# chenjiaoAngel/Paddle-Lite

Hardware: AMD Instinct MI355X
Metric: INT8 images/sec MobileNetV1 224x224 (higher is better)
Workload: dtype int8; 1 GPU; MobileNetV1 INT8 full graph 224x224 (27 int8 convs + pool + fc + softmax), random-init weights, 128 images per step and GPU (4 predictors / HIP streams, each running whole steps: 4 steps in flight), input resident in HBM; steps_in_flight=4, global_batch=128

## Files before the change

paddle-lite_amd/csrc/conv_stem_common.h:

```cpp
#pragma once
#include <type_traits>

#include "gemm_epilogue.h"
#include "gemm_tr_common.h"
#include "plhip_kernels.h"

namespace plhip {

constexpr int STEM_LDS_PITCH = 272;

inline dim3 stem_grid(const DirectS2Args& a) {
  const long nblk = (long)(((a.ow >> 2) + 31) / 32) * ((a.oh + 3) / 4) * a.n;
  return dim3((unsigned)((nblk + 7) / 8 * 8));
}

template <class F>
inline void stem_dispatch(const DirectS2Args& a, int out, F&& launch) {
  using std::integral_constant;
  const bool mfull = a.cout % 32 == 0;
#define PLHIP_STEM(O)                                                                \
  do {                                                                               \
    if (mfull) launch(integral_constant<int, O>{}, integral_constant<bool, true>{}); \
    else launch(integral_constant<int, O>{}, integral_constant<bool, false>{});      \
  } while (0)
  if (out == OUT_I32) PLHIP_STEM(OUT_I32);
  else if (out == OUT_F32) PLHIP_STEM(OUT_F32);
  else PLHIP_STEM(OUT_I8);
#undef PLHIP_STEM
}

__device__ __forceinline__ bool stem_block(const DirectS2Args& a, int& bx, int& by, int& b) {
  const int nx = ((a.ow >> 2) + 31) >> 5, ny = (a.oh + 3) >> 2;
  const unsigned nb = (unsigned)(nx * ny * a.n), per = (nb + 7) >> 3;
  const unsigned vb = (blockIdx.x & 7) * per + (blockIdx.x >> 3);
  bx = (int)(vb % (unsigned)nx);
  const unsigned t = vb / (unsigned)nx;
  by = (int)(t % (unsigned)ny);
  b = (int)(t / (unsigned)ny);
  return vb < nb;
}

template <bool TAIL>
__device__ __forceinline__ void stem_gemm_args(const DirectS2Args& a, GemmArgs& g) {
  g.y = a.y;
  g.scale = a.scale;
  g.bias = a.bias;
  g.M = a.cout;
  g.HWY = a.oh * a.ow;
  g.y_bstride = (size_t)a.cout * a.oh * a.ow;
  g.act = a.act;
  g.alpha = a.alpha;
  g.res = TAIL ? a.res : nullptr;
  g.res_relu = TAIL ? a.res_relu : 0;
  g.y2 = TAIL ? a.y2 : nullptr;
  g.inv_scale2 = TAIL ? a.inv_scale2 : 0.f;
}

template <int OUT>
__device__ __forceinline__ v4i stem3x3_begin(const DirectS2Args& a, const int8_t* __restrict__ afrag, int lane, float* lsb,
                                             GemmArgs& g) {
  stem_gemm_args<false>(a, g);
  const v4i af0 = *reinterpret_cast<const v4i*>(afrag + (size_t)lane * 16);
  if (OUT != OUT_I32) stage_scale_bias<1, OUT>(g, 0, lane, lsb);
  return af0;
}

__device__ __forceinline__ void stem3x3_lds_windows(const uint8_t* img, int cin, int lane, int wave, uint32_t (&win)[4][5]) {
  const int c = lane & 31, h = lane >> 5;
#pragma unroll
  for (int L = 0; L < 5; ++L) {
    const int cr = 5 * h + L;
    const int ci = cr / 3, r3 = cr - ci * 3;
    const bool live = cr < 3 * cin;
    const int lrow = live ? ci * 9 + 2 * wave + r3 : 0;
    const uint8_t* p = img + lrow * STEM_LDS_PITCH + 8 * c;
    const v2i lo = *reinterpret_cast<const v2i*>(p), hi = *reinterpret_cast<const v2i*>(p + 8);
    const uint32_t m = live ? 0xffffffffu : 0u;
    const uint32_t d0 = (uint32_t)lo[0] & m, d1 = (uint32_t)lo[1] & m, d2 = (uint32_t)hi[0] & m, d3 = (uint32_t)hi[1] & m;
    win[0][L] = __builtin_amdgcn_alignbyte(d1, d0, 3);
    win[1][L] = __builtin_amdgcn_alignbyte(d2, d1, 1);
    win[2][L] = __builtin_amdgcn_alignbyte(d2, d1, 3);
    win[3][L] = __builtin_amdgcn_alignbyte(d3, d2, 1);
  }
}

template <int OUT, bool MFULL>
__device__ __forceinline__ void stem3x3_mfma(const GemmArgs g, const int8_t* __restrict__ afrag, v4i af0, const uint32_t (&win)[4][5],
                                             float* lsb, int lane, int b, int hw, bool qvalid) {
  const int h = lane >> 5;
  v4i bf[4];
#pragma unroll
  for (int j = 0; j < 4; ++j) {
    bf[j][0] = (int)__builtin_amdgcn_perm(win[j][1], win[j][0], 0x04020100u);
    bf[j][1] = (int)__builtin_amdgcn_perm(win[j][2], win[j][1], 0x05040201u);
    bf[j][2] = (int)__builtin_amdgcn_perm(win[j][3], win[j][2], 0x06050402u);
    bf[j][3] = (int)(win[j][4] & 0x00ffffffu);
  }
  const int MT = (g.M + 31) >> 5;
  for (int mt = 0; mt < MT; ++mt) {
    v4i af = af0;
    if (mt > 0) {
      af = *reinterpret_cast<const v4i*>(afrag + ((size_t)mt * 64 + lane) * 16);
      if (OUT != OUT_I32) stage_scale_bias<1, OUT>(g, mt, lane, lsb);
    }
    v16i acc[1][4];
    const v16i zero16 = {0, 0, 0, 0, 0, 0, 0, 0, 0, 0, 0, 0, 0, 0, 0, 0};
#pragma unroll
    for (int j = 0; j < 4; ++j) acc[0][j] = __builtin_amdgcn_mfma_i32_32x32x32_i8(af, bf[j], zero16, 0, 0, 0);
    if (qvalid) gemm_epilogue_act<1, OUT, true, MFULL>(g, acc, mt, h, b, hw, lsb, g.HWY - hw);
  }
}

template <int OUT, bool MFULL>
__device__ __forceinline__ void stem3x3_staged(const DirectS2Args& a, const int8_t* __restrict__ afrag, const uint8_t* img, float* lsb,
                                               int lane, int wave, int bx, int by, int b) {
  const int owq = a.ow >> 2;
  const int oy = by * 4 + wave;
  int xq = bx * 32 + (lane & 31);
  const bool qvalid = xq < owq && oy < a.oh;
  if (xq >= owq) xq = owq - 1;

  GemmArgs g;
  const v4i af0 = stem3x3_begin<OUT>(a, afrag, lane, lsb, g);
  __syncthreads();

  uint32_t win[4][5];
  stem3x3_lds_windows(img, a.cin, lane, wave, win);
  stem3x3_mfma<OUT, MFULL>(g, afrag, af0, win, lsb, lane, b, oy * a.ow + 4 * xq, qvalid);
}

}
```

paddle-lite_amd/csrc/conv_stem_f32in.hip:

```cpp
#include "conv_stem_common.h"

namespace plhip {

bool conv3x3s2_f32in_supported(const DirectS2Args& a) {
  return a.cin >= 1 && a.cin <= 3 && (a.ow & 3) == 0 && (a.w & 3) == 0 && a.pl == 1 && (a.pt == 0 || a.pt == 1) && a.cout <= 128 &&
         (long)a.n * a.cin * a.h * a.w < (1L << 31) && (long)(((a.ow >> 2) + 31) / 32) * ((a.oh + 3) / 4) * a.n < (1L << 31) - 8;
}

template <int OUT, bool MFULL>
__global__ __launch_bounds__(256) void conv3x3s2_mfma_f32in_kernel(DirectS2Args a, const int8_t* __restrict__ afrag) {
  PLHIP_PRELOAD(a.xf); PLHIP_PRELOAD(a.y); PLHIP_PRELOAD(a.scale); PLHIP_PRELOAD(a.bias); PLHIP_PRELOAD(afrag);
  PLHIP_PRELOAD(a.n); PLHIP_PRELOAD(a.cin); PLHIP_PRELOAD(a.h); PLHIP_PRELOAD(a.w); PLHIP_PRELOAD(a.cout); PLHIP_PRELOAD(a.oh);
  PLHIP_PRELOAD(a.ow); PLHIP_PRELOAD(a.pt); PLHIP_PRELOAD(a.act); PLHIP_PRELOAD(a.alpha); PLHIP_PRELOAD(a.x_inv_scale);
  __shared__ __attribute__((aligned(16))) float lsb_all[4][64];
  __shared__ __attribute__((aligned(16))) uint8_t img[27 * STEM_LDS_PITCH];
  const int lane = threadIdx.x & 63;
  const int wave = __builtin_amdgcn_readfirstlane((int)(threadIdx.x >> 6));
  float* lsb = lsb_all[wave];
  int bx, by, b;
  if (!stem_block(a, bx, by, b)) return;

  const int c0 = 256 * bx - 4, ih0 = 8 * by - a.pt;
  const int nrows = a.cin * 9;
  const float inv = a.x_inv_scale;
  const size_t img_base = (size_t)b * a.cin * a.h * a.w;
  constexpr int NPIECE = (27 * 66 + 255) / 256;
  v4f pv[NPIECE];
  int pdst[NPIECE];
#pragma unroll
  for (int it = 0; it < NPIECE; ++it) {
    const int k = it * 256 + (int)threadIdx.x;
    const int row = k / 66, piece = k - row * 66;
    const int ci = row / 9, j = row - ci * 9;
    const int ih = ih0 + j, col = c0 + 4 * piece;
    pdst[it] = k < nrows * 66 ? row * STEM_LDS_PITCH + 4 * piece : -1;
    pv[it] = v4f{0.f, 0.f, 0.f, 0.f};
    if (k < nrows * 66 && ih >= 0 && ih < a.h && col >= 0 && col < a.w)
      pv[it] = *reinterpret_cast<const v4f*>(a.xf + img_base + ((size_t)ci * a.h + ih) * a.w + col);
  }
#pragma unroll
  for (int it = 0; it < NPIECE; ++it) {
    const v4f v = pv[it];
    const uint32_t pk = pack4_i8(round_sat_i8(inv * v[0]), round_sat_i8(inv * v[1]), round_sat_i8(inv * v[2]), round_sat_i8(inv * v[3]));
    if (pdst[it] >= 0) *reinterpret_cast<uint32_t*>(img + pdst[it]) = pk;
  }

  stem3x3_staged<OUT, MFULL>(a, afrag, img, lsb, lane, wave, bx, by, b);
}

void launch_conv3x3s2_f32in(const DirectS2Args& a, const int8_t* afrag, int out, hipStream_t s) {
  stem_dispatch(a, out, [&](auto O, auto MF) {
    hipLaunchKernelGGL((conv3x3s2_mfma_f32in_kernel<decltype(O)::value, decltype(MF)::value>), stem_grid(a), dim3(256), 0, s, a, afrag);
  });
}

}
```

paddle-lite_amd/csrc/conv_stem_u8in.hip:

```cpp
#include "conv_stem_common.h"

namespace plhip {

bool conv3x3s2_u8in_supported(const DirectS2Args& a, const ImageArgs& im) {
  return conv3x3s2_f32in_supported(a) && (im.cs == 1 || im.cs == 3 || im.cs == 4) && im.c == (im.cs == 1 ? 1 : 3) && a.cin == im.c &&
         im.n == a.n && im.h == a.h && im.w == a.w && (long)a.n * a.h * a.w * im.cs < (1L << 31);
}

template <int OUT, bool MFULL, int CS>
__global__ __launch_bounds__(256) void conv3x3s2_mfma_u8in_kernel(DirectS2Args a, ImageArgs im, const int8_t* __restrict__ afrag) {
  PLHIP_PRELOAD(im.src); PLHIP_PRELOAD(a.y); PLHIP_PRELOAD(a.scale); PLHIP_PRELOAD(a.bias); PLHIP_PRELOAD(afrag);
  PLHIP_PRELOAD(a.n); PLHIP_PRELOAD(a.cin); PLHIP_PRELOAD(a.h); PLHIP_PRELOAD(a.w); PLHIP_PRELOAD(a.cout); PLHIP_PRELOAD(a.oh);
  PLHIP_PRELOAD(a.ow); PLHIP_PRELOAD(a.pt); PLHIP_PRELOAD(a.act); PLHIP_PRELOAD(a.alpha); PLHIP_PRELOAD(a.x_inv_scale);
  constexpr int C = CS == 1 ? 1 : 3;
  __shared__ __attribute__((aligned(16))) float lsb_all[4][64];
  __shared__ __attribute__((aligned(16))) uint8_t img[27 * STEM_LDS_PITCH];
  const int lane = threadIdx.x & 63;
  const int wave = __builtin_amdgcn_readfirstlane((int)(threadIdx.x >> 6));
  float* lsb = lsb_all[wave];
  int bx, by, b;
  if (!stem_block(a, bx, by, b)) return;

  const int c0 = 256 * bx - 4, ih0 = 8 * by - a.pt;
  const float inv = a.x_inv_scale;
  constexpr int NPIECE = (9 * 66 + 255) / 256;
  uint32_t pw[NPIECE][CS];
  int pdst[NPIECE];
  bool pin[NPIECE];
#pragma unroll
  for (int it = 0; it < NPIECE; ++it) {
    const int k = it * 256 + (int)threadIdx.x;
    const int j = k / 66, piece = k - j * 66;
    const int ih = ih0 + j, col = c0 + 4 * piece;
    pdst[it] = k < 9 * 66 ? j * STEM_LDS_PITCH + 4 * piece : -1;
    pin[it] = k < 9 * 66 && ih >= 0 && ih < a.h && col >= 0 && col < a.w;
#pragma unroll
    for (int d = 0; d < CS; ++d) pw[it][d] = 0u;
    if (pin[it]) {
      const uint32_t* p = reinterpret_cast<const uint32_t*>(im.src + (((size_t)b * a.h + ih) * a.w + col) * CS);
#pragma unroll
      for (int d = 0; d < CS; ++d) pw[it][d] = p[d];
    }
  }
#pragma unroll
  for (int it = 0; it < NPIECE; ++it) {
#pragma unroll
    for (int ci = 0; ci < C; ++ci) {
      int q[4];
#pragma unroll
      for (int e = 0; e < 4; ++e) {
        const int bi = e * CS + ci;
        const float u = (float)((pw[it][bi >> 2] >> (8 * (bi & 3))) & 0xffu);
        q[e] = round_sat_i8(inv * ((u - im.mean[ci]) * im.scale[ci]));
      }
      const uint32_t pk = pin[it] ? pack4_i8(q[0], q[1], q[2], q[3]) : 0u;
      if (pdst[it] >= 0) *reinterpret_cast<uint32_t*>(img + ci * 9 * STEM_LDS_PITCH + pdst[it]) = pk;
    }
  }

  stem3x3_staged<OUT, MFULL>(a, afrag, img, lsb, lane, wave, bx, by, b);
}

template <int CS>
static void launch_u8in_cs(const DirectS2Args& a, const ImageArgs& im, const int8_t* afrag, int out, hipStream_t s) {
  stem_dispatch(a, out, [&](auto O, auto MF) {
    hipLaunchKernelGGL((conv3x3s2_mfma_u8in_kernel<decltype(O)::value, decltype(MF)::value, CS>), stem_grid(a), dim3(256), 0, s, a, im, afrag);
  });
}

void launch_conv3x3s2_u8in(const DirectS2Args& a, const ImageArgs& im, const int8_t* afrag, int out, hipStream_t s) {
  if (im.cs == 1) launch_u8in_cs<1>(a, im, afrag, out, s);
  else if (im.cs == 3) launch_u8in_cs<3>(a, im, afrag, out, s);
  else launch_u8in_cs<4>(a, im, afrag, out, s);
}

}
```

paddle-lite_amd/csrc/misc_ops.hip:

```cpp
#include <stdlib.h>

#include "plhip_device.h"
#include "plhip_kernels.h"

namespace plhip {

__device__ __forceinline__ float mul_then_add_two_roundings(float a, float s, float b) {
#pragma clang fp contract(off)
  const float p = a * s;
  return p + b;
}
__device__ __forceinline__ float fc_epilogue_f32(int acc, float s, float b, int flags) {
  float y = (flags & 2) ? mul_then_add_two_roundings((float)acc, s, b) : __fmaf_rn((float)acc, s, b);
  if (flags & 1) y = y > 0.f ? y : 0.f;
  return y;
}

__global__ void pack_fc_kernel(const int8_t* __restrict__ w, int8_t* __restrict__ wp, int k, int n) {
  const int k4n = (k + 3) / 4;
  const size_t total = (size_t)k4n * n * 4;
  for (size_t idx = (size_t)blockIdx.x * blockDim.x + threadIdx.x; idx < total; idx += (size_t)gridDim.x * blockDim.x) {
    const int j = idx & 3;
    const size_t t = idx >> 2;
    const int col = (int)(t % n);
    const int kq = (int)(t / n);
    const int kk = kq * 4 + j;
    wp[idx] = kk < k ? w[(size_t)kk * n + col] : (int8_t)0;
  }
}

#define FC_MB 8
template <int OUT>
__global__ __launch_bounds__(256) void fc_i8_kernel(const int8_t* __restrict__ x, const int8_t* __restrict__ wp,
                                                    const float* __restrict__ scale, const float* __restrict__ bias,
                                                    void* __restrict__ y, int m, int k, int n, int relu) {
  const int col = blockIdx.x * 256 + threadIdx.x;
  const int m0 = blockIdx.y * FC_MB;
  const int k4n = (k + 3) / 4;
  int acc[FC_MB];
#pragma unroll
  for (int i = 0; i < FC_MB; ++i) acc[i] = 0;
  const int colc = col < n ? col : n - 1;
  const uint32_t* wq = reinterpret_cast<const uint32_t*>(wp) + colc;
  for (int kq = 0; kq < k4n; ++kq) {
    const int wv = (int)wq[(size_t)kq * n];
#pragma unroll
    for (int i = 0; i < FC_MB; ++i) {
      const int mi = m0 + i < m ? m0 + i : m - 1;
      const int8_t* xr = x + (size_t)mi * k + kq * 4;
      uint32_t xv = 0;
      if (kq * 4 + 3 < k) {
        __builtin_memcpy(&xv, xr, 4);
      } else {
        for (int j = 0; j < 4; ++j)
          if (kq * 4 + j < k) xv |= (uint32_t)(uint8_t)xr[j] << (8 * j);
      }
      acc[i] = __builtin_amdgcn_sdot4((int)xv, wv, acc[i], false);
    }
  }
  if (col >= n) return;
  const float s = (OUT == OUT_I32) ? 1.f : scale[col];
  const float bi = (OUT != OUT_I32 && bias) ? bias[col] : 0.f;
#pragma unroll
  for (int i = 0; i < FC_MB; ++i) {
    if (m0 + i >= m) break;
    const size_t off = (size_t)(m0 + i) * n + col;
    if (OUT == OUT_I32) {
      reinterpret_cast<int*>(y)[off] = acc[i];
    } else {
      const float f = fc_epilogue_f32(acc[i], s, bi, relu);
      if (OUT == OUT_F32) reinterpret_cast<float*>(y)[off] = f;
      else reinterpret_cast<int8_t*>(y)[off] = (int8_t)round_sat_i8(f);
    }
  }
}

#define FCF_MB 16
template <int OUT>
__global__ __launch_bounds__(256) void fc_i8_fast_kernel(const int8_t* __restrict__ x, const int8_t* __restrict__ wp,
                                                         const float* __restrict__ scale, const float* __restrict__ bias,
                                                         void* __restrict__ y, int m, int k, int n, int relu) {
  extern __shared__ __attribute__((aligned(16))) uint8_t fsm[];
  const int lane = threadIdx.x & 63;
  const int wave = __builtin_amdgcn_readfirstlane(threadIdx.x >> 6);
  const int col = blockIdx.x * 64 + lane;
  const int m0 = blockIdx.y * FCF_MB;
  const int k4n = k >> 2;
  const int k16n = k >> 4;
  {
    const v4i* src = reinterpret_cast<const v4i*>(x);
    v4i* dst = reinterpret_cast<v4i*>(fsm);
    for (int i = threadIdx.x; i < FCF_MB * k16n; i += 256) {
      const int r = i / k16n, c16 = i - r * k16n;
      const int mi = m0 + r < m ? m0 + r : m - 1;
      dst[i] = src[(size_t)mi * k16n + c16];
    }
  }
  __syncthreads();
  const int g0 = (k16n * wave) / 4, g1 = (k16n * (wave + 1)) / 4;
  const int colc = col < n ? col : n - 1;
  const uint32_t* wq = reinterpret_cast<const uint32_t*>(wp) + colc;
  int acc[FCF_MB];
#pragma unroll
  for (int i = 0; i < FCF_MB; ++i) acc[i] = 0;
  for (int gq = g0; gq < g1; ++gq) {
    int wv[4];
#pragma unroll
    for (int u = 0; u < 4; ++u) wv[u] = (int)wq[(size_t)(gq * 4 + u) * n];
#pragma unroll
    for (int i = 0; i < FCF_MB; ++i) {
      const v4i xv = *reinterpret_cast<const v4i*>(fsm + ((size_t)i * k16n + gq) * 16);
#pragma unroll
      for (int u = 0; u < 4; ++u) acc[i] = __builtin_amdgcn_sdot4(xv[u], wv[u], acc[i], false);
    }
  }
  __syncthreads();
  int* red = reinterpret_cast<int*>(fsm);
#pragma unroll
  for (int i = 0; i < FCF_MB; ++i) red[(wave * FCF_MB + i) * 64 + lane] = acc[i];
  __syncthreads();
  if (col >= n) return;
  const float s = (OUT == OUT_I32) ? 1.f : scale[col];
  const float bi = (OUT != OUT_I32 && bias) ? bias[col] : 0.f;
#pragma unroll
  for (int j = 0; j < FCF_MB / 4; ++j) {
    const int i = wave * (FCF_MB / 4) + j;
    if (m0 + i >= m) break;
    const int a = red[(0 * FCF_MB + i) * 64 + lane] + red[(1 * FCF_MB + i) * 64 + lane] + red[(2 * FCF_MB + i) * 64 + lane] +
                  red[(3 * FCF_MB + i) * 64 + lane];
    const size_t off = (size_t)(m0 + i) * n + col;
    if (OUT == OUT_I32) {
      reinterpret_cast<int*>(y)[off] = a;
    } else {
      const float f = fc_epilogue_f32(a, s, bi, relu);
      if (OUT == OUT_F32) reinterpret_cast<float*>(y)[off] = f;
      else reinterpret_cast<int8_t*>(y)[off] = (int8_t)round_sat_i8(f);
    }
  }
}

size_t fc_dot4_bytes(int k, int n) { return (((size_t)((k + 3) / 4) * n * 4) + 15) & ~(size_t)15; }
size_t fc_packed_bytes(int k, int n) { return fc_dot4_bytes(k, n) + (size_t)((n + 31) / 32) * ((k + 31) / 32) * 1024; }

__global__ void pack_fc_mfma_kernel(const int8_t* __restrict__ w, int8_t* __restrict__ wp, int k, int n) {
  const int KS = (k + 31) / 32;
  const size_t total = (size_t)((n + 31) / 32) * KS * 1024;
  for (size_t idx = (size_t)blockIdx.x * blockDim.x + threadIdx.x; idx < total; idx += (size_t)gridDim.x * blockDim.x) {
    const int j = idx & 15, lane = (idx >> 4) & 63;
    const size_t t = idx >> 10;
    const int ks = (int)(t % KS), nt = (int)(t / KS);
    const int nn = nt * 32 + (lane & 31), kk = ks * 32 + 16 * (lane >> 5) + j;
    wp[idx] = (nn < n && kk < k) ? w[(size_t)kk * n + nn] : (int8_t)0;
  }
}

template <int OUT>
__global__ __launch_bounds__(256) void fc_i8_mfma_kernel(const int8_t* __restrict__ x, const int8_t* __restrict__ wfrag,
                                                         const float* __restrict__ scale, const float* __restrict__ bias,
                                                         void* __restrict__ y, int m, int k, int n, int relu) {
  __shared__ int red[4][16][64];
  const int lane = threadIdx.x & 63;
  const int wave = __builtin_amdgcn_readfirstlane((int)(threadIdx.x >> 6));
  const int c = lane & 31, h = lane >> 5;
  const int nt = blockIdx.x, mt = blockIdx.y;
  const int KS = k >> 5;
  const int ks0 = (KS * wave) >> 2, ks1 = (KS * (wave + 1)) >> 2;
  const int mrow = mt * 32 + c < m ? mt * 32 + c : m - 1;
  const int8_t* xb = x + (size_t)mrow * k + 16 * h;
  const int8_t* ab = wfrag + (size_t)nt * KS * 1024 + lane * 16;
  const int n0 = nt * 32 + 8 * wave + 4 * h;
  v16i acc;
#pragma unroll
  for (int r = 0; r < 16; ++r) acc[r] = 0;
  for (int ks = ks0; ks < ks1; ks += 8) {
    v4i af[8], bf[8];
#pragma unroll
    for (int u = 0; u < 8; ++u) {
      const int kk = ks + u < ks1 ? ks + u : ks1 - 1;
      af[u] = *reinterpret_cast<const v4i*>(ab + (size_t)kk * 1024);
      __builtin_memcpy(&bf[u], xb + (size_t)kk * 32, 16);
    }
#pragma unroll
    for (int u = 0; u < 8; ++u)
      if (ks + u < ks1) acc = __builtin_amdgcn_mfma_i32_32x32x32_i8(af[u], bf[u], acc, 0, 0, 0);
  }
#pragma unroll
  for (int r = 0; r < 16; ++r) red[wave][r][lane] = acc[r];
  __syncthreads();
  const int mcol = mt * 32 + c;
  if (mcol >= m || n0 >= n) return;
  float sc4[4] = {1.f, 1.f, 1.f, 1.f}, bi4[4] = {0.f, 0.f, 0.f, 0.f};
  if (OUT != OUT_I32) {
#pragma unroll
    for (int e = 0; e < 4; ++e) sc4[e] = scale[n0 + e < n ? n0 + e : n - 1];
    if (bias) {
#pragma unroll
      for (int e = 0; e < 4; ++e) bi4[e] = bias[n0 + e < n ? n0 + e : n - 1];
    }
  }
  float f[4];
  int a4[4];
#pragma unroll
  for (int e = 0; e < 4; ++e) {
    const int r = 4 * wave + e;
    a4[e] = (red[0][r][lane] + red[1][r][lane]) + (red[2][r][lane] + red[3][r][lane]);
    f[e] = fc_epilogue_f32(a4[e], sc4[e], bi4[e], relu);
  }
  const size_t off = (size_t)mcol * n + n0;
  const int cnt = n - n0 < 4 ? n - n0 : 4;
  if (OUT == OUT_I32) {
    int* yp = reinterpret_cast<int*>(y) + off;
    if (cnt == 4) __builtin_memcpy(yp, a4, 16);
    else for (int e = 0; e < cnt; ++e) yp[e] = a4[e];
  } else if (OUT == OUT_F32) {
    float* yp = reinterpret_cast<float*>(y) + off;
    if (cnt == 4) __builtin_memcpy(yp, f, 16);
    else for (int e = 0; e < cnt; ++e) yp[e] = f[e];
  } else {
    int8_t* yp = reinterpret_cast<int8_t*>(y) + off;
    const uint32_t pk = pack4_i8(round_sat_i8(f[0]), round_sat_i8(f[1]), round_sat_i8(f[2]), round_sat_i8(f[3]));
    if (cnt == 4) __builtin_memcpy(yp, &pk, 4);
    else for (int e = 0; e < cnt; ++e) yp[e] = (int8_t)(pk >> (8 * e));
  }
}

__global__ void calib_f32_to_i8_kernel(const float* __restrict__ x, int8_t* __restrict__ y, float inv_scale, int64_t count, int vec) {
  const int64_t nq = vec ? count >> 2 : 0;
  const int64_t stride = (int64_t)gridDim.x * blockDim.x;
  for (int64_t i = (int64_t)blockIdx.x * blockDim.x + threadIdx.x; i < nq; i += stride) {
    const v4f v = reinterpret_cast<const v4f*>(x)[i];
    reinterpret_cast<uint32_t*>(y)[i] = pack4_i8(round_sat_i8(inv_scale * v[0]), round_sat_i8(inv_scale * v[1]),
                                                 round_sat_i8(inv_scale * v[2]), round_sat_i8(inv_scale * v[3]));
  }
  for (int64_t t = (nq << 2) + (int64_t)blockIdx.x * blockDim.x + threadIdx.x; t < count; t += stride)
    y[t] = (int8_t)round_sat_i8(inv_scale * x[t]);
}

__global__ void calib_i8_to_f32_kernel(const int8_t* __restrict__ x, float* __restrict__ y, float scale, int64_t count, int vec) {
  const int64_t nq = vec ? count >> 2 : 0;
  const int64_t stride = (int64_t)gridDim.x * blockDim.x;
  for (int64_t i = (int64_t)blockIdx.x * blockDim.x + threadIdx.x; i < nq; i += stride) {
    const uint32_t v = reinterpret_cast<const uint32_t*>(x)[i];
    v4f o;
    o[0] = scale * (float)(int8_t)(v & 0xff);
    o[1] = scale * (float)(int8_t)((v >> 8) & 0xff);
    o[2] = scale * (float)(int8_t)((v >> 16) & 0xff);
    o[3] = scale * (float)(int8_t)(v >> 24);
    reinterpret_cast<v4f*>(y)[i] = o;
  }
  for (int64_t t = (nq << 2) + (int64_t)blockIdx.x * blockDim.x + threadIdx.x; t < count; t += stride)
    y[t] = scale * (float)x[t];
}

__global__ __launch_bounds__(256) void global_avg_pool_kernel(const float* __restrict__ x, int nc, int spatial, float* __restrict__ y) {
  const int sub = threadIdx.x & 15;
  const int plane = blockIdx.x * 16 + (threadIdx.x >> 4);
  float s = 0.f;
  if (plane < nc) {
    const float* p = x + (size_t)plane * spatial;
    for (int i = sub; i < spatial; i += 16) s += p[i];
  }
#pragma unroll
  for (int off = 8; off > 0; off >>= 1) s += __shfl_xor(s, off, 16);
  if (sub == 0 && plane < nc) y[plane] = s / (float)spatial;
}

__global__ __launch_bounds__(256) void softmax_kernel(const float* __restrict__ x, int cols, float* __restrict__ y) {
  __shared__ float red[4];
  const float* xr = x + (size_t)blockIdx.x * cols;
  float* yr = y + (size_t)blockIdx.x * cols;
  const int lane = threadIdx.x & 63, wave = threadIdx.x >> 6;
  float mx = -3.402823466e38f;
  for (int i = threadIdx.x; i < cols; i += 256) mx = fmaxf(mx, xr[i]);
#pragma unroll
  for (int off = 32; off > 0; off >>= 1) mx = fmaxf(mx, __shfl_down(mx, off, 64));
  if (lane == 0) red[wave] = mx;
  __syncthreads();
  mx = fmaxf(fmaxf(red[0], red[1]), fmaxf(red[2], red[3]));
  __syncthreads();
  float s = 0.f;
  for (int i = threadIdx.x; i < cols; i += 256) s += expf(xr[i] - mx);
#pragma unroll
  for (int off = 32; off > 0; off >>= 1) s += __shfl_down(s, off, 64);
  if (lane == 0) red[wave] = s;
  __syncthreads();
  s = (red[0] + red[1]) + (red[2] + red[3]);
  for (int i = threadIdx.x; i < cols; i += 256) yr[i] = expf(xr[i] - mx) / s;
}

void launch_pack_fc(const int8_t* w_kn, int8_t* wp, int k, int n, hipStream_t s) {
  const size_t total = (size_t)((k + 3) / 4) * n * 4;
  size_t blocks = (total + 255) / 256;
  if (blocks > 4096) blocks = 4096;
  hipLaunchKernelGGL(pack_fc_kernel, dim3((unsigned)blocks), dim3(256), 0, s, w_kn, wp, k, n);
  const size_t ftotal = (size_t)((n + 31) / 32) * ((k + 31) / 32) * 1024;
  size_t fblocks = (ftotal + 255) / 256;
  if (fblocks > 4096) fblocks = 4096;
  hipLaunchKernelGGL(pack_fc_mfma_kernel, dim3((unsigned)fblocks), dim3(256), 0, s, w_kn, wp + fc_dot4_bytes(k, n), k, n);
}

void launch_fc(const int8_t* x, const int8_t* wp, const float* scale, const float* bias, void* y, int m, int k, int n,
               int relu, int out, hipStream_t s) {
  const int fc_mfma_env = knob("FC_MFMA", 0);
  const size_t lds_f = (size_t)FCF_MB * k > (size_t)4 * FCF_MB * 64 * 4 ? (size_t)FCF_MB * k : (size_t)4 * FCF_MB * 64 * 4;
  const bool fast_ok = (k & 15) == 0 && ((uintptr_t)x & 15) == 0 && lds_f <= 64 * 1024;
  if ((fc_mfma_env || !fast_ok) && (k & 31) == 0) {
    dim3 grid((n + 31) / 32, (m + 31) / 32);
    const int8_t* wfrag = wp + fc_dot4_bytes(k, n);
    if (out == OUT_I32) hipLaunchKernelGGL((fc_i8_mfma_kernel<OUT_I32>), grid, dim3(256), 0, s, x, wfrag, scale, bias, y, m, k, n, relu);
    else if (out == OUT_F32) hipLaunchKernelGGL((fc_i8_mfma_kernel<OUT_F32>), grid, dim3(256), 0, s, x, wfrag, scale, bias, y, m, k, n, relu);
    else hipLaunchKernelGGL((fc_i8_mfma_kernel<OUT_I8>), grid, dim3(256), 0, s, x, wfrag, scale, bias, y, m, k, n, relu);
    return;
  }
  const size_t lds = (size_t)FCF_MB * k > (size_t)4 * FCF_MB * 64 * 4 ? (size_t)FCF_MB * k : (size_t)4 * FCF_MB * 64 * 4;
  if ((k & 15) == 0 && ((uintptr_t)x & 15) == 0 && lds <= 64 * 1024) {
    dim3 grid((n + 63) / 64, (m + FCF_MB - 1) / FCF_MB);
    if (out == OUT_I32) hipLaunchKernelGGL((fc_i8_fast_kernel<OUT_I32>), grid, dim3(256), lds, s, x, wp, scale, bias, y, m, k, n, relu);
    else if (out == OUT_F32) hipLaunchKernelGGL((fc_i8_fast_kernel<OUT_F32>), grid, dim3(256), lds, s, x, wp, scale, bias, y, m, k, n, relu);
    else hipLaunchKernelGGL((fc_i8_fast_kernel<OUT_I8>), grid, dim3(256), lds, s, x, wp, scale, bias, y, m, k, n, relu);
    return;
  }
  dim3 grid((n + 255) / 256, (m + FC_MB - 1) / FC_MB);
  if (out == OUT_I32) hipLaunchKernelGGL((fc_i8_kernel<OUT_I32>), grid, dim3(256), 0, s, x, wp, scale, bias, y, m, k, n, relu);
  else if (out == OUT_F32) hipLaunchKernelGGL((fc_i8_kernel<OUT_F32>), grid, dim3(256), 0, s, x, wp, scale, bias, y, m, k, n, relu);
  else hipLaunchKernelGGL((fc_i8_kernel<OUT_I8>), grid, dim3(256), 0, s, x, wp, scale, bias, y, m, k, n, relu);
}

static unsigned ew_blocks(int64_t quads) {
  int64_t b = (quads + 255) / 256;
  if (b < 1) b = 1;
  if (b > 2048 * 4) b = 2048 * 4;
  return (unsigned)b;
}

void launch_calib_f32_to_i8(const float* x, int8_t* y, float scale, int64_t count, hipStream_t s) {
  const float inv = 1.f / scale;
  const int vec = (((uintptr_t)x & 15) == 0 && ((uintptr_t)y & 3) == 0) ? 1 : 0;
  hipLaunchKernelGGL(calib_f32_to_i8_kernel, dim3(ew_blocks(vec ? count >> 2 : count)), dim3(256), 0, s, x, y, inv, count, vec);
}

void launch_calib_i8_to_f32(const int8_t* x, float* y, float scale, int64_t count, hipStream_t s) {
  const int vec = (((uintptr_t)y & 15) == 0 && ((uintptr_t)x & 3) == 0) ? 1 : 0;
  hipLaunchKernelGGL(calib_i8_to_f32_kernel, dim3(ew_blocks(vec ? count >> 2 : count)), dim3(256), 0, s, x, y, scale, count, vec);
}

void launch_global_avg_pool(const float* x, int nc, int spatial, float* y, hipStream_t s) {
  hipLaunchKernelGGL(global_avg_pool_kernel, dim3((nc + 15) / 16), dim3(256), 0, s, x, nc, spatial, y);
}

void launch_softmax(const float* x, int rows, int cols, float* y, hipStream_t s) {
  hipLaunchKernelGGL(softmax_kernel, dim3(rows), dim3(256), 0, s, x, cols, y);
}

}
```

Measured before the change: 415,400 img/s.

## Restructure stem tile staging and pipeline FC weight loads with adaptive row blocking

The stem conv input staging is refactored into a templated request/convert source abstraction. Each wave loads whole rows plus edge pieces, and the scale/bias loads are issued before the tile conversion, so global loads overlap with the quantize-and-store step. The fast FC kernel now prefetches activations into registers in batches and loads weights in groups of 16 ahead of the dot products. It also gains an 8-row block variant, picked when the grid would have fewer than 256 blocks, to raise parallelism. The cost is more register pressure and more template instantiations.

Measured after the change: 418,900 img/s (median of 4 runs). Within noise of the previous version (+0.8%).

```diff
diff --git a/paddle-lite_amd/csrc/conv_stem_common.h b/paddle-lite_amd/csrc/conv_stem_common.h
--- a/paddle-lite_amd/csrc/conv_stem_common.h
+++ b/paddle-lite_amd/csrc/conv_stem_common.h
@@ -111,19 +111,66 @@
   }
 }
 
-template <int OUT, bool MFULL>
-__device__ __forceinline__ void stem3x3_staged(const DirectS2Args& a, const int8_t* __restrict__ afrag, const uint8_t* img, float* lsb,
+template <class SRC>
+struct StemPieces {
+  static constexpr int SLOTS = (SRC::SETS * 9 + 3) / 4;
+  typename SRC::Piece main[SLOTS], edge;
+};
+
+template <class SRC>
+__device__ __forceinline__ void stem3x3_request(const DirectS2Args& a, const SRC& src, int b, int bx, int by, int lane, int wave,
+                                                StemPieces<SRC>& pc) {
+  const int c0 = 256 * bx - 4, ih0 = 8 * by - a.pt, sets = src.sets();
+#pragma unroll
+  for (int it = 0; it < StemPieces<SRC>::SLOTS; ++it) {
+    const int r = it * 4 + wave, set = r / 9, ih = ih0 + (r - set * 9), col = c0 + 4 * (lane + 1);
+    pc.main[it] = SRC::zero();
+    if (set < sets && ih >= 0 && ih < a.h) {
+      const auto* row = src.row(b, set, ih);
+      if (col < a.w) pc.main[it] = src.fetch(row, col);
+    }
+  }
+  const int r = (int)threadIdx.x >> 1, set = r / 9, ih = ih0 + (r - set * 9), col = c0 + ((threadIdx.x & 1) ? 260 : 0);
+  pc.edge = SRC::zero();
+  if (set < sets && ih >= 0 && ih < a.h && col >= 0 && col < a.w) pc.edge = src.fetch(src.row(b, set, ih), col);
+}
+
+template <class SRC>
+__device__ __forceinline__ void stem3x3_convert(const DirectS2Args& a, const SRC& src, int bx, int by, int lane, int wave, uint8_t* tile,
+                                                const StemPieces<SRC>& pc) {
+  const int c0 = 256 * bx - 4, ih0 = 8 * by - a.pt, sets = src.sets();
+#pragma unroll
+  for (int it = 0; it < StemPieces<SRC>::SLOTS; ++it) SRC::await(pc.main[it]);
+  SRC::await(pc.edge);
+#pragma unroll
+  for (int it = 0; it < StemPieces<SRC>::SLOTS; ++it) {
+    const int r = it * 4 + wave, set = r / 9, j = r - set * 9, ih = ih0 + j, col = c0 + 4 * (lane + 1);
+    if (set < sets) src.put(tile, set, j, lane + 1, pc.main[it], ih >= 0 && ih < a.h && col < a.w);
+  }
+  const int r = (int)threadIdx.x >> 1, set = r / 9, j = r - set * 9, ih = ih0 + j, p = (threadIdx.x & 1) ? 65 : 0, col = c0 + 4 * p;
+  if (set < sets) src.put(tile, set, j, p, pc.edge, ih >= 0 && ih < a.h && col >= 0 && col < a.w);
+}
+
+constexpr int STEM_TILE_BYTES = 27 * STEM_LDS_PITCH;
+template <int OUT, bool MFULL, class SRC>
+__device__ __forceinline__ void stem3x3_staged(const DirectS2Args& a, const SRC& src, const int8_t* __restrict__ afrag, uint8_t* img, float* lsb,
                                                int lane, int wave, int bx, int by, int b) {
+  GemmArgs g;
+  stem_gemm_args<false>(a, g);
+  const v4i af0 = *reinterpret_cast<const v4i*>(afrag + (size_t)lane * 16);
+  float s0 = 1.f, b0 = 0.f;
+  if (OUT != OUT_I32) load_scale_bias<1>(g, 0, lane, s0, b0);
+  StemPieces<SRC> pc;
+  stem3x3_request(a, src, b, bx, by, lane, wave, pc);
+  stem3x3_convert(a, src, bx, by, lane, wave, img, pc);
+  if (OUT != OUT_I32) store_scale_bias<1, OUT>(lsb, lane, s0, b0);
+  __syncthreads();
+
   const int owq = a.ow >> 2;
   const int oy = by * 4 + wave;
   int xq = bx * 32 + (lane & 31);
   const bool qvalid = xq < owq && oy < a.oh;
   if (xq >= owq) xq = owq - 1;
-
-  GemmArgs g;
-  const v4i af0 = stem3x3_begin<OUT>(a, afrag, lane, lsb, g);
-  __syncthreads();
-
   uint32_t win[4][5];
   stem3x3_lds_windows(img, a.cin, lane, wave, win);
   stem3x3_mfma<OUT, MFULL>(g, afrag, af0, win, lsb, lane, b, oy * a.ow + 4 * xq, qvalid);
diff --git a/paddle-lite_amd/csrc/conv_stem_f32in.hip b/paddle-lite_amd/csrc/conv_stem_f32in.hip
--- a/paddle-lite_amd/csrc/conv_stem_f32in.hip
+++ b/paddle-lite_amd/csrc/conv_stem_f32in.hip
@@ -7,45 +7,36 @@
          (long)a.n * a.cin * a.h * a.w < (1L << 31) && (long)(((a.ow >> 2) + 31) / 32) * ((a.oh + 3) / 4) * a.n < (1L << 31) - 8;
 }
 
+struct StemSrcF32 {
+  static constexpr int SETS = 3;
+  using Piece = v4f;
+  const float* __restrict__ x;
+  int cin, h, w;
+  float inv;
+  __device__ __forceinline__ int sets() const { return cin; }
+  static __device__ __forceinline__ Piece zero() { return v4f{0.f, 0.f, 0.f, 0.f}; }
+  __device__ __forceinline__ const float* row(int b, int set, int ih) const { return x + ((size_t)(b * cin + set) * h + ih) * w; }
+  static __device__ __forceinline__ Piece fetch(const float* row, int col) { return *reinterpret_cast<const v4f*>(row + (unsigned)col); }
+  static __device__ __forceinline__ void await(const Piece& v) { asm volatile("" ::"v"(v)); }
+  __device__ __forceinline__ void put(uint8_t* tile, int set, int j, int p, const Piece& v, bool) const {
+    *reinterpret_cast<uint32_t*>(tile + (set * 9 + j) * STEM_LDS_PITCH + 4 * p) =
+        pack4_i8(round_sat_i8(inv * v[0]), round_sat_i8(inv * v[1]), round_sat_i8(inv * v[2]), round_sat_i8(inv * v[3]));
+  }
+};
+
 template <int OUT, bool MFULL>
 __global__ __launch_bounds__(256) void conv3x3s2_mfma_f32in_kernel(DirectS2Args a, const int8_t* __restrict__ afrag) {
   PLHIP_PRELOAD(a.xf); PLHIP_PRELOAD(a.y); PLHIP_PRELOAD(a.scale); PLHIP_PRELOAD(a.bias); PLHIP_PRELOAD(afrag);
   PLHIP_PRELOAD(a.n); PLHIP_PRELOAD(a.cin); PLHIP_PRELOAD(a.h); PLHIP_PRELOAD(a.w); PLHIP_PRELOAD(a.cout); PLHIP_PRELOAD(a.oh);
   PLHIP_PRELOAD(a.ow); PLHIP_PRELOAD(a.pt); PLHIP_PRELOAD(a.act); PLHIP_PRELOAD(a.alpha); PLHIP_PRELOAD(a.x_inv_scale);
   __shared__ __attribute__((aligned(16))) float lsb_all[4][64];
-  __shared__ __attribute__((aligned(16))) uint8_t img[27 * STEM_LDS_PITCH];
+  __shared__ __attribute__((aligned(16))) uint8_t img[STEM_TILE_BYTES];
   const int lane = threadIdx.x & 63;
   const int wave = __builtin_amdgcn_readfirstlane((int)(threadIdx.x >> 6));
-  float* lsb = lsb_all[wave];
   int bx, by, b;
   if (!stem_block(a, bx, by, b)) return;
-
-  const int c0 = 256 * bx - 4, ih0 = 8 * by - a.pt;
-  const int nrows = a.cin * 9;
-  const float inv = a.x_inv_scale;
-  const size_t img_base = (size_t)b * a.cin * a.h * a.w;
-  constexpr int NPIECE = (27 * 66 + 255) / 256;
-  v4f pv[NPIECE];
-  int pdst[NPIECE];
-#pragma unroll
-  for (int it = 0; it < NPIECE; ++it) {
-    const int k = it * 256 + (int)threadIdx.x;
-    const int row = k / 66, piece = k - row * 66;
-    const int ci = row / 9, j = row - ci * 9;
-    const int ih = ih0 + j, col = c0 + 4 * piece;
-    pdst[it] = k < nrows * 66 ? row * STEM_LDS_PITCH + 4 * piece : -1;
-    pv[it] = v4f{0.f, 0.f, 0.f, 0.f};
-    if (k < nrows * 66 && ih >= 0 && ih < a.h && col >= 0 && col < a.w)
-      pv[it] = *reinterpret_cast<const v4f*>(a.xf + img_base + ((size_t)ci * a.h + ih) * a.w + col);
-  }
-#pragma unroll
-  for (int it = 0; it < NPIECE; ++it) {
-    const v4f v = pv[it];
-    const uint32_t pk = pack4_i8(round_sat_i8(inv * v[0]), round_sat_i8(inv * v[1]), round_sat_i8(inv * v[2]), round_sat_i8(inv * v[3]));
-    if (pdst[it] >= 0) *reinterpret_cast<uint32_t*>(img + pdst[it]) = pk;
-  }
-
-  stem3x3_staged<OUT, MFULL>(a, afrag, img, lsb, lane, wave, bx, by, b);
+  const StemSrcF32 src = {a.xf, a.cin, a.h, a.w, a.x_inv_scale};
+  stem3x3_staged<OUT, MFULL>(a, src, afrag, img, lsb_all[wave], lane, wave, bx, by, b);
 }
 
 void launch_conv3x3s2_f32in(const DirectS2Args& a, const int8_t* afrag, int out, hipStream_t s) {
diff --git a/paddle-lite_amd/csrc/conv_stem_u8in.hip b/paddle-lite_amd/csrc/conv_stem_u8in.hip
--- a/paddle-lite_amd/csrc/conv_stem_u8in.hip
+++ b/paddle-lite_amd/csrc/conv_stem_u8in.hip
@@ -7,58 +7,61 @@
          im.n == a.n && im.h == a.h && im.w == a.w && (long)a.n * a.h * a.w * im.cs < (1L << 31);
 }
 
-template <int OUT, bool MFULL, int CS>
-__global__ __launch_bounds__(256) void conv3x3s2_mfma_u8in_kernel(DirectS2Args a, ImageArgs im, const int8_t* __restrict__ afrag) {
-  PLHIP_PRELOAD(im.src); PLHIP_PRELOAD(a.y); PLHIP_PRELOAD(a.scale); PLHIP_PRELOAD(a.bias); PLHIP_PRELOAD(afrag);
-  PLHIP_PRELOAD(a.n); PLHIP_PRELOAD(a.cin); PLHIP_PRELOAD(a.h); PLHIP_PRELOAD(a.w); PLHIP_PRELOAD(a.cout); PLHIP_PRELOAD(a.oh);
-  PLHIP_PRELOAD(a.ow); PLHIP_PRELOAD(a.pt); PLHIP_PRELOAD(a.act); PLHIP_PRELOAD(a.alpha); PLHIP_PRELOAD(a.x_inv_scale);
-  constexpr int C = CS == 1 ? 1 : 3;
-  __shared__ __attribute__((aligned(16))) float lsb_all[4][64];
-  __shared__ __attribute__((aligned(16))) uint8_t img[27 * STEM_LDS_PITCH];
-  const int lane = threadIdx.x & 63;
-  const int wave = __builtin_amdgcn_readfirstlane((int)(threadIdx.x >> 6));
-  float* lsb = lsb_all[wave];
-  int bx, by, b;
-  if (!stem_block(a, bx, by, b)) return;
-
-  const int c0 = 256 * bx - 4, ih0 = 8 * by - a.pt;
-  const float inv = a.x_inv_scale;
-  constexpr int NPIECE = (9 * 66 + 255) / 256;
-  uint32_t pw[NPIECE][CS];
-  int pdst[NPIECE];
-  bool pin[NPIECE];
+template <int CS>
+struct StemSrcU8 {
+  static constexpr int SETS = 1;
+  static constexpr int C = CS == 1 ? 1 : 3;
+  struct Piece { uint32_t d[CS]; };
+  const uint8_t* __restrict__ img;
+  int h, w;
+  float inv, mean[3], scale[3];
+  __device__ __forceinline__ int sets() const { return 1; }
+  static __device__ __forceinline__ Piece zero() {
+    Piece v;
 #pragma unroll
-  for (int it = 0; it < NPIECE; ++it) {
-    const int k = it * 256 + (int)threadIdx.x;
-    const int j = k / 66, piece = k - j * 66;
-    const int ih = ih0 + j, col = c0 + 4 * piece;
-    pdst[it] = k < 9 * 66 ? j * STEM_LDS_PITCH + 4 * piece : -1;
-    pin[it] = k < 9 * 66 && ih >= 0 && ih < a.h && col >= 0 && col < a.w;
+    for (int d = 0; d < CS; ++d) v.d[d] = 0u;
+    return v;
+  }
+  __device__ __forceinline__ const uint8_t* row(int b, int, int ih) const { return img + ((size_t)b * h + ih) * w * CS; }
+  static __device__ __forceinline__ Piece fetch(const uint8_t* row, int col) {
+    const uint32_t* p = reinterpret_cast<const uint32_t*>(row + (unsigned)col * CS);
+    Piece v;
 #pragma unroll
-    for (int d = 0; d < CS; ++d) pw[it][d] = 0u;
-    if (pin[it]) {
-      const uint32_t* p = reinterpret_cast<const uint32_t*>(im.src + (((size_t)b * a.h + ih) * a.w + col) * CS);
+    for (int d = 0; d < CS; ++d) v.d[d] = p[d];
+    return v;
+  }
+  static __device__ __forceinline__ void await(const Piece& v) {
 #pragma unroll
-      for (int d = 0; d < CS; ++d) pw[it][d] = p[d];
-    }
+    for (int d = 0; d < CS; ++d) asm volatile("" ::"v"(v.d[d]));
   }
-#pragma unroll
-  for (int it = 0; it < NPIECE; ++it) {
+  __device__ __forceinline__ void put(uint8_t* tile, int, int j, int p, const Piece& v, bool inside) const {
 #pragma unroll
     for (int ci = 0; ci < C; ++ci) {
       int q[4];
 #pragma unroll
       for (int e = 0; e < 4; ++e) {
         const int bi = e * CS + ci;
-        const float u = (float)((pw[it][bi >> 2] >> (8 * (bi & 3))) & 0xffu);
-        q[e] = round_sat_i8(inv * ((u - im.mean[ci]) * im.scale[ci]));
+        const float u = (float)((v.d[bi >> 2] >> (8 * (bi & 3))) & 0xffu);
+        q[e] = round_sat_i8(inv * ((u - mean[ci]) * scale[ci]));
       }
-      const uint32_t pk = pin[it] ? pack4_i8(q[0], q[1], q[2], q[3]) : 0u;
-      if (pdst[it] >= 0) *reinterpret_cast<uint32_t*>(img + ci * 9 * STEM_LDS_PITCH + pdst[it]) = pk;
+      *reinterpret_cast<uint32_t*>(tile + (ci * 9 + j) * STEM_LDS_PITCH + 4 * p) = inside ? pack4_i8(q[0], q[1], q[2], q[3]) : 0u;
     }
   }
+};
 
-  stem3x3_staged<OUT, MFULL>(a, afrag, img, lsb, lane, wave, bx, by, b);
+template <int OUT, bool MFULL, int CS>
+__global__ __launch_bounds__(256) void conv3x3s2_mfma_u8in_kernel(DirectS2Args a, ImageArgs im, const int8_t* __restrict__ afrag) {
+  PLHIP_PRELOAD(im.src); PLHIP_PRELOAD(a.y); PLHIP_PRELOAD(a.scale); PLHIP_PRELOAD(a.bias); PLHIP_PRELOAD(afrag);
+  PLHIP_PRELOAD(a.n); PLHIP_PRELOAD(a.cin); PLHIP_PRELOAD(a.h); PLHIP_PRELOAD(a.w); PLHIP_PRELOAD(a.cout); PLHIP_PRELOAD(a.oh);
+  PLHIP_PRELOAD(a.ow); PLHIP_PRELOAD(a.pt); PLHIP_PRELOAD(a.act); PLHIP_PRELOAD(a.alpha); PLHIP_PRELOAD(a.x_inv_scale);
+  __shared__ __attribute__((aligned(16))) float lsb_all[4][64];
+  __shared__ __attribute__((aligned(16))) uint8_t img[STEM_TILE_BYTES];
+  const int lane = threadIdx.x & 63;
+  const int wave = __builtin_amdgcn_readfirstlane((int)(threadIdx.x >> 6));
+  int bx, by, b;
+  if (!stem_block(a, bx, by, b)) return;
+  const StemSrcU8<CS> src = {im.src, a.h, a.w, a.x_inv_scale, {im.mean[0], im.mean[1], im.mean[2]}, {im.scale[0], im.scale[1], im.scale[2]}};
+  stem3x3_staged<OUT, MFULL>(a, src, afrag, img, lsb_all[wave], lane, wave, bx, by, b);
 }
 
 template <int CS>
diff --git a/paddle-lite_amd/csrc/misc_ops.hip b/paddle-lite_amd/csrc/misc_ops.hip
--- a/paddle-lite_amd/csrc/misc_ops.hip
+++ b/paddle-lite_amd/csrc/misc_ops.hip
@@ -76,7 +76,9 @@
 }
 
 #define FCF_MB 16
-template <int OUT>
+constexpr int FCF_XP = 8;
+constexpr int FCF_WG = 16;
+template <int OUT, int MB>
 __global__ __launch_bounds__(256) void fc_i8_fast_kernel(const int8_t* __restrict__ x, const int8_t* __restrict__ wp,
                                                          const float* __restrict__ scale, const float* __restrict__ bias,
                                                          void* __restrict__ y, int m, int k, int n, int relu) {
@@ -84,50 +86,86 @@
   const int lane = threadIdx.x & 63;
   const int wave = __builtin_amdgcn_readfirstlane(threadIdx.x >> 6);
   const int col = blockIdx.x * 64 + lane;
-  const int m0 = blockIdx.y * FCF_MB;
-  const int k4n = k >> 2;
+  const int m0 = blockIdx.y * MB;
   const int k16n = k >> 4;
-  {
-    const v4i* src = reinterpret_cast<const v4i*>(x);
-    v4i* dst = reinterpret_cast<v4i*>(fsm);
-    for (int i = threadIdx.x; i < FCF_MB * k16n; i += 256) {
-      const int r = i / k16n, c16 = i - r * k16n;
-      const int mi = m0 + r < m ? m0 + r : m - 1;
-      dst[i] = src[(size_t)mi * k16n + c16];
-    }
-  }
-  __syncthreads();
+  const int colc = col < n ? col : n - 1;
+  const float s = (OUT == OUT_I32) ? 1.f : scale[colc];
+  const float bi = (OUT != OUT_I32 && bias) ? bias[colc] : 0.f;
+  const v4i* src = reinterpret_cast<const v4i*>(x);
+  v4i* dst = reinterpret_cast<v4i*>(fsm);
+  const size_t x0 = (size_t)m0 * k16n;
+  const int xlive = (m - m0 < MB ? m - m0 : MB) * k16n;
+  v4i xp[FCF_XP];
+#pragma unroll
+  for (int u = 0; u < FCF_XP; ++u) {
+    const int i = u * 256 + (int)threadIdx.x;
+    xp[u] = src[x0 + (i < xlive ? i : xlive - 1)];
+  }
   const int g0 = (k16n * wave) / 4, g1 = (k16n * (wave + 1)) / 4;
-  const int colc = col < n ? col : n - 1;
-  const uint32_t* wq = reinterpret_cast<const uint32_t*>(wp) + colc;
-  int acc[FCF_MB];
-#pragma unroll
-  for (int i = 0; i < FCF_MB; ++i) acc[i] = 0;
-  for (int gq = g0; gq < g1; ++gq) {
-    int wv[4];
-#pragma unroll
-    for (int u = 0; u < 4; ++u) wv[u] = (int)wq[(size_t)(gq * 4 + u) * n];
-#pragma unroll
-    for (int i = 0; i < FCF_MB; ++i) {
-      const v4i xv = *reinterpret_cast<const v4i*>(fsm + ((size_t)i * k16n + gq) * 16);
-#pragma unroll
-      for (int u = 0; u < 4; ++u) acc[i] = __builtin_amdgcn_sdot4(xv[u], wv[u], acc[i], false);
-    }
+  const uint32_t* wq = reinterpret_cast<const uint32_t*>(wp);
+  int wv[FCF_WG][4];
+  auto request_w = [&](int gb) {
+#pragma unroll
+    for (int c = 0; c < FCF_WG; ++c) {
+      int gq = gb + c < g1 ? gb + c : g1 - 1;
+      gq = gq < 0 ? 0 : gq;
+#pragma unroll
+      for (int u = 0; u < 4; ++u) wv[c][u] = (int)(wq + (size_t)(gq * 4 + u) * n)[(unsigned)colc];
+    }
+  };
+  request_w(g0);
+#pragma unroll
+  for (int u = 0; u < FCF_XP; ++u) {
+    const int i = u * 256 + (int)threadIdx.x;
+    if (i < xlive) dst[i] = xp[u];
+  }
+  for (int i0 = FCF_XP * 256; i0 < xlive; i0 += FCF_XP * 256) {
+#pragma unroll
+    for (int u = 0; u < FCF_XP; ++u) {
+      const int i = i0 + u * 256 + (int)threadIdx.x;
+      xp[u] = src[x0 + (i < xlive ? i : xlive - 1)];
+    }
+#pragma unroll
+    for (int u = 0; u < FCF_XP; ++u) {
+      const int i = i0 + u * 256 + (int)threadIdx.x;
+      if (i < xlive) dst[i] = xp[u];
+    }
+  }
+  __syncthreads();
+  int acc[MB];
+#pragma unroll
+  for (int i = 0; i < MB; ++i) acc[i] = 0;
+  auto dot_w = [&](int gb) {
+#pragma unroll
+    for (int c = 0; c < FCF_WG; ++c) {
+      const int gq = gb + c;
+      if (gq < g1) {
+#pragma unroll
+        for (int i = 0; i < MB; ++i) {
+          const v4i xv = *reinterpret_cast<const v4i*>(fsm + ((size_t)i * k16n + gq) * 16);
+#pragma unroll
+          for (int u = 0; u < 4; ++u) acc[i] = __builtin_amdgcn_sdot4(xv[u], wv[c][u], acc[i], false);
+        }
+      }
+    }
+  };
+  dot_w(g0);
+  for (int gb = g0 + FCF_WG; gb < g1; gb += FCF_WG) {
+    request_w(gb);
+    dot_w(gb);
   }
   __syncthreads();
   int* red = reinterpret_cast<int*>(fsm);
 #pragma unroll
-  for (int i = 0; i < FCF_MB; ++i) red[(wave * FCF_MB + i) * 64 + lane] = acc[i];
+  for (int i = 0; i < MB; ++i) red[(wave * MB + i) * 64 + lane] = acc[i];
   __syncthreads();
   if (col >= n) return;
-  const float s = (OUT == OUT_I32) ? 1.f : scale[col];
-  const float bi = (OUT != OUT_I32 && bias) ? bias[col] : 0.f;
-#pragma unroll
-  for (int j = 0; j < FCF_MB / 4; ++j) {
-    const int i = wave * (FCF_MB / 4) + j;
+#pragma unroll
+  for (int j = 0; j < MB / 4; ++j) {
+    const int i = wave * (MB / 4) + j;
     if (m0 + i >= m) break;
-    const int a = red[(0 * FCF_MB + i) * 64 + lane] + red[(1 * FCF_MB + i) * 64 + lane] + red[(2 * FCF_MB + i) * 64 + lane] +
-                  red[(3 * FCF_MB + i) * 64 + lane];
+    const int a = red[(0 * MB + i) * 64 + lane] + red[(1 * MB + i) * 64 + lane] + red[(2 * MB + i) * 64 + lane] +
+                  red[(3 * MB + i) * 64 + lane];
     const size_t off = (size_t)(m0 + i) * n + col;
     if (OUT == OUT_I32) {
       reinterpret_cast<int*>(y)[off] = a;
@@ -312,12 +350,19 @@
     else hipLaunchKernelGGL((fc_i8_mfma_kernel<OUT_I8>), grid, dim3(256), 0, s, x, wfrag, scale, bias, y, m, k, n, relu);
     return;
   }
-  const size_t lds = (size_t)FCF_MB * k > (size_t)4 * FCF_MB * 64 * 4 ? (size_t)FCF_MB * k : (size_t)4 * FCF_MB * 64 * 4;
-  if ((k & 15) == 0 && ((uintptr_t)x & 15) == 0 && lds <= 64 * 1024) {
-    dim3 grid((n + 63) / 64, (m + FCF_MB - 1) / FCF_MB);
-    if (out == OUT_I32) hipLaunchKernelGGL((fc_i8_fast_kernel<OUT_I32>), grid, dim3(256), lds, s, x, wp, scale, bias, y, m, k, n, relu);
-    else if (out == OUT_F32) hipLaunchKernelGGL((fc_i8_fast_kernel<OUT_F32>), grid, dim3(256), lds, s, x, wp, scale, bias, y, m, k, n, relu);
-    else hipLaunchKernelGGL((fc_i8_fast_kernel<OUT_I8>), grid, dim3(256), lds, s, x, wp, scale, bias, y, m, k, n, relu);
+  if (fast_ok) {
+    const int mb = (long)((n + 63) / 64) * ((m + FCF_MB - 1) / FCF_MB) < 256 ? 8 : FCF_MB;
+    const size_t lds = (size_t)mb * k > (size_t)4 * mb * 64 * 4 ? (size_t)mb * k : (size_t)4 * mb * 64 * 4;
+    dim3 grid((n + 63) / 64, (m + mb - 1) / mb);
+#define PLHIP_FC_FAST(O)                                                                                                              \
+  do {                                                                                                                                \
+    if (mb == 8) hipLaunchKernelGGL((fc_i8_fast_kernel<O, 8>), grid, dim3(256), lds, s, x, wp, scale, bias, y, m, k, n, relu);         \
+    else hipLaunchKernelGGL((fc_i8_fast_kernel<O, FCF_MB>), grid, dim3(256), lds, s, x, wp, scale, bias, y, m, k, n, relu);           \
+  } while (0)
+    if (out == OUT_I32) PLHIP_FC_FAST(OUT_I32);
+    else if (out == OUT_F32) PLHIP_FC_FAST(OUT_F32);
+    else PLHIP_FC_FAST(OUT_I8);
+#undef PLHIP_FC_FAST
     return;
   }
   dim3 grid((n + 255) / 256, (m + FC_MB - 1) / FC_MB);
```
